# ElenaBiagi/Finito

Hardware: AMD Instinct MI355X
Metric: localized k-mers/s (k=31) (higher is better)
Workload: dtype u32

## Files before the change

### finito_amd/csrc/fin_capi.cpp

```cpp
#include <functional>
#include <hip/hip_runtime_api.h>
#include <sched.h>

#include <algorithm>
#include <atomic>
#include <chrono>
#include <condition_variable>
#include <cstdio>
#include <cstdlib>
#include <cstring>
#include <memory>
#include <mutex>
#include <new>
#include <string>
#include <thread>
#include <vector>

#include "../../include/finito_amd.h"
#include "fin_index.hpp"
#include "fin_kernels.h"

static void set_err(char* err, size_t errlen, const std::string& msg) {
    if (err && errlen) { snprintf(err, errlen, "%s", msg.c_str()); }
}
// ... 28 lines not shown
        if (hipHostMalloc(&p, want, hipHostMallocDefault) != hipSuccess) return nullptr;
        *cap = want;
        return p;
    }
    void put(void* p, size_t cap) {
        if (!p) return;
        {
            std::lock_guard<std::mutex> g(mu);
            if (free_list.size() < 8 && held + cap <= (4ull << 30)) { free_list.push_back({p, cap}); held += cap; return; }
        }
        (void)hipHostFree(p);
    }
    void release_all() {
        std::lock_guard<std::mutex> g(mu);
        for (auto& f : free_list) (void)hipHostFree(f.first);
        free_list.clear(); held = 0;
    }
};
StagePool g_stage;
bool is_page_locked(const void* p) {
    if (!p) return true;
    hipPointerAttribute_t a;
    memset(&a, 0, sizeof a);
    if (hipPointerGetAttributes(&a, p) != hipSuccess) { (void)hipGetLastError(); return false; }
    return a.type == hipMemoryTypeHost;
}
}

extern "C" {

const char* fin_version(void) { return "finito-amd 0.1 (gfx950)"; }

enum : int { O_lds_deque_limit, O_kernel, O_probe_prepass, O_ptab_t, O_jtab_t, O_write_gaps, O_overlap_prefill, O_filt_f, O_seed_anchors, O_kmer_table,
              O_defer_strand, O_fast_path, O_cbf_m, O_lean_tables, O_text_anchors, O_epoch_budget_mult, O_epoch_budget_add, O_max_batch_kmers, O_pipeline_kmers, O_pipeline_depth, O_stage_pageable, O_debug_ovf_cap, O_debug_pp_seg, O_lean_walk, O_fused_ingest, O_pp_park, O_debug_pp_park_cap, O_pp_wide_out, O_hits_combine, O_cover_probe, O_debug_depth_tile, O_ec_tag_bits, O_ec_combine, O_COUNT };
static_assert(O_COUNT <= FIN_N_OPTIONS, "fin_index::opt_val has room for every option");
struct OptDef { const char* name; int64_t def, lo, hi; };
static const OptDef OPTS[O_COUNT] = {
    {"lds_deque_limit", 16, 1, 16},
    {"kernel", 4, 0, 4},
    {"probe_prepass", 1, 0, 1},
    {"ptab_t", -1, -1, 15},
    {"jtab_t", -1, -1, 14},
    {"write_gaps", 1, 0, 1},
    {"overlap_prefill", 1, 0, 1},
    {"filt_f", -1, -1, 16},
    {"seed_anchors", 1, 0, 1},
    {"kmer_table", 1, 0, 1},
    {"defer_strand", 1, 0, 1},
    {"fast_path", 1, 0, 2},
    {"cbf_m", -1, -1, 32},
    {"lean_tables", 2, 0, 3},
    {"text_anchors", 1, 0, 1},
    {"epoch_budget_mult", 64, 0, 64},
    {"epoch_budget_add", 4096, 1, 1 << 20},
    {"max_batch_kmers", 1ll << 30, 1, 1ll << 31},
    {"pipeline_kmers", 1ll << 26, 1, 1ll << 31},
    {"pipeline_depth", 3, 1, 8},
    {"stage_pageable", 1, 0, 1},
    {"debug_ovf_cap", 0, 0, 1ll << 31},
    {"debug_pp_seg", 0, 0, 1024},
    {"lean_walk", 1, 0, 1},
    {"fused_ingest", 1, 0, 1},
    {"pp_park", 1, 0, 1},
    {"debug_pp_park_cap", -1, -1, 1024},
    {"pp_wide_out", 1, 0, 1},
    {"hits_combine", 4, 0, 64},
    {"cover_probe", 0, 0, 1},
    {"debug_depth_tile", 0, 0, 4096},
    {"ec_tag_bits", 63, 1, 63},
    {"ec_combine", 1, 0, 1},
};
static std::atomic<int64_t> g_opt[O_COUNT];
static const bool g_opt_init = [] { for (int i = 0; i < O_COUNT; i++) g_opt[i].store(OPTS[i].def); return true; }();
static inline int64_t optv(const fin_index* x, int id) { return x && x->opt_set[id].load(std::memory_order_acquire) ? x->opt_val[id].load(std::memory_order_relaxed) : g_opt[id].load(std::memory_order_relaxed); }
static int opt_find(const char* name, int64_t value) {
    if (!name) return -1;
    for (int i = 0; i < O_COUNT; i++)
        if (!strcmp(name, OPTS[i].name)) return (value < OPTS[i].lo || value > OPTS[i].hi || (i == O_kernel && value == 1)) ? -1 : i;
    return -1;
}

int fin_set_option(const char* name, int64_t value) {
    (void)g_opt_init;
    const int id = opt_find(name, value);
    if (id < 0) return FIN_EINVAL;
    g_opt[id].store(value);
    if (id == O_stage_pageable && !value) g_stage.release_all();
    return FIN_OK;
}

int fin_index_set_option(fin_index* idx, const char* name, int64_t value) {
    if (!idx) return FIN_EINVAL;
    const int id = opt_find(name, value);
    if (id < 0) return FIN_EINVAL;
    idx->opt_val[id].store(value, std::memory_order_relaxed); idx->opt_set[id].store(true, std::memory_order_release);
    return FIN_OK;
}

// ... 707 lines not shown
    const int rc = batch_load(b, bases ? bases + offsets[0] : nullptr, offsets, n_reads, err, errlen);
    if (rc != FIN_OK) { fin_batch_free(b); return rc; }
    *out = b;
    return FIN_OK;
}

int fin_batch_reload(fin_batch* b, const char* bases, const uint64_t* offsets, uint64_t n_reads, char* err, size_t errlen) {
    if (!b || !offsets || (n_reads && !bases)) { set_err(err, errlen, "null argument"); return FIN_EINVAL; }
    return batch_load(b, bases ? bases + offsets[0] : nullptr, offsets, n_reads, err, errlen);
}

int fin_batch_run(fin_batch* b, int strands, void* hip_stream, char* err, size_t errlen) {
    if (!b || (strands != FIN_FWD && strands != FIN_MERGED)) { set_err(err, errlen, "bad argument"); return FIN_EINVAL; }
    HIPCHK(hipSetDevice(b->device));
    hipStream_t st = (hipStream_t)hip_stream;
    if (b->runs.size() >= 1024) {
        for (auto& e : b->runs.front().e) (void)hipEventDestroy(e);
        b->runs.erase(b->runs.begin());
    }
    fin_batch::RunEvents ev;
    for (auto& e : ev.e) HIPCHK(hipEventCreate(&e));
    b->runs.push_back(ev);
    b->last_strands = strands;
    b->last_stream = st; b->ran = true;
    HIPCHK(hipEventRecord(ev.e[0], st));
    b->dev.budget_mult = (uint32_t)optv(b->idx, O_epoch_budget_mult); b->dev.budget_add = (uint32_t)optv(b->idx, O_epoch_budget_add);
    b->dev.ovf_cap = (uint32_t)std::min<uint64_t>(b->cap_ovf_list / 4, 0xFFFFFFFFull);
    if (const int64_t forced = optv(b->idx, O_debug_ovf_cap)) b->dev.ovf_cap = (uint32_t)std::min<int64_t>(forced, (int64_t)b->dev.ovf_cap);
    b->last_ovf_cap = b->dev.ovf_cap; b->ovf_state = 0; b->rec_ready = false; b->sgm_ready = false; b->rsum_ready = false; b->scr_ready = false; b->cls_ready = false; b->psa_ready = false;
    b->dev.pp_seg = (uint32_t)optv(b->idx, O_debug_pp_seg);
    b->dev.pp_max_len = (uint32_t)std::min<uint64_t>(b->max_read_len, 0xFFFFFFFFull);
    b->dev.pp_park = (uint32_t)optv(b->idx, O_pp_park);
    b->dev.pp_wide_out = (uint32_t)optv(b->idx, O_pp_wide_out);
    b->dev.pp_park_cap = (uint32_t)(int32_t)optv(b->idx, O_debug_pp_park_cap);
    b->dev.lean_walk = (uint32_t)optv(b->idx, O_lean_walk);
    {
        const fin_index::Replica* rep = b->idx->replica_on(b->device);
        b->dev.text_anchors = (optv(b->idx, O_text_anchors) && rep && rep->anchors_built) ? 1u : 0u;
        b->dev.safe = rep ? rep->dev.safe : nullptr;
        b->dev.pos = (optv(b->idx, O_seed_anchors) && b->dev.text_anchors && b->d_seed && rep) ? rep->dev.pos : nullptr;
        b->dev.filt = (optv(b->idx, O_filt_f) != 0 && rep) ? rep->dev.filt : nullptr;
        const bool lean = rep && rep->lean && optv(b->idx, O_seed_anchors) && b->dev.text_anchors && b->d_seed && optv(b->idx, O_kmer_table) && rep->dev.fbf;
        b->dev.fbf = lean ? rep->dev.fbf : nullptr;
        b->dev.kt3 = (optv(b->idx, O_kmer_table) && rep && (b->dev.pos || lean)) ? rep->dev.kt3 : nullptr;
        b->dev.ktx = (b->dev.kt3 && rep) ? rep->dev.ktx : nullptr; b->dev.ktx_log2 = rep ? rep->dev.ktx_log2 : 0;
        b->dev.cbf = (rep && b->dev.kt3) ? rep->dev.cbf : nullptr;
        b->dev.fast_path = (optv(b->idx, O_fast_path) && b->dev.cbf) ? 1u : 0u;
    }
    int rc = 0;
    hipEvent_t out_ready = nullptr;
    const int opt_kernel = (int)optv(b->idx, O_kernel);
    const uint32_t lds_limit = (uint32_t)optv(b->idx, O_lds_deque_limit);
    int kern = opt_kernel;
    if (b->dev.k > FIN_FAST_K)
        kern = (opt_kernel == 4 && b->q_slots && fin_v4_writes_gaps(&b->dev, (const uint32_t*)b->d_seed)) ? 4 : 0;
    const int no_prefill = (kern == 4 && b->q_slots && optv(b->idx, O_write_gaps) && fin_v4_writes_gaps(&b->dev, (const uint32_t*)b->d_seed)) ? 1 : 0;
    {
        const fin_index::Replica* rep = b->idx->replica_on(b->device);
        b->dev.defer_ok = (kern == 4 && no_prefill && strands == FIN_MERGED && optv(b->idx, O_defer_strand) && rep && rep->anchors_built &&
                           rep->n_rc_pairs != ~0ull && (b->dev.pos || b->dev.fbf)) ? 1u : 0u;
        b->dev.rcwin = (b->dev.defer_ok && rep->d_rcwin) ? (const uint8_t*)rep->d_rcwin : nullptr;
    }
    b->last_kernel = (uint32_t)((kern == 4 && !b->q_slots) ? 3 : kern); b->last_no_prefill = (uint32_t)no_prefill;
    if (!(b->dev.defer_ok && b->dev.kt3 && (b->dev.k <= 63 || optv(b->idx, O_fast_path) >= 2))) b->dev.fast_path = 0u;
    b->dev.frec = nullptr; b->dev.text_only = 0u; b->last_frec = false; b->last_text_only = false; b->count_from_text = false;
    if (b->text_mode && kern == 4 && b->q_slots && b->dev.fast_path && no_prefill && strands == FIN_MERGED && b->n_reads) {
// ... 2713 lines not shown
```

### finito_amd/csrc/fin_format.h

```cpp
#pragma once
#include <stdint.h>

#define FIN_BLOCK_NODES 64
#define FIN_LCS_MASK 0x7Fu
#define FIN_USTART_BIT 0x80u
#define FIN_MAX_K 255
#define FIN_FAST_K 128

struct FinCharRec {
    uint32_t plane_lo, plane_hi;
    uint32_t base;
};
struct alignas(128) FinNodeBlock {
    uint8_t node[64];
    FinCharRec rec[4];
    uint64_t th0, th1;
};
static_assert(sizeof(FinNodeBlock) == 128, "one block = one 128-B line");
#ifdef __HIPCC__
__host__ __device__
#endif
static inline uint64_t fin_plane(const FinCharRec& r) { return r.plane_lo | ((uint64_t)r.plane_hi << 32); }

struct FinBlockInfo {
// ... 14 lines not shown
    uint32_t n_nodes;
    uint32_t n_unitigs;
    uint32_t total_len;
    uint32_t k;
    uint32_t samp_shift;
    uint32_t n_samp;
    uint32_t C[5];
    uint32_t lcs_t0;
    uint32_t ptab_t;
    const struct FinPrefixIval* ptab;
    uint32_t jtab_t;
    const struct FinPrefixIval* jtab;
    uint32_t budget_mult, budget_add;
    uint32_t ovf_cap;
    uint32_t text_anchors;
    const struct FinSeedEntry* pos;
    const unsigned long long* safe;
    const struct FinKt3Bucket* kt3;
    uint32_t kt3_buckets;
    const struct FinKtxSlot* ktx;
    uint32_t ktx_log2;
    const struct FinCbfBlock* cbf;
    uint32_t cbf_log2, cbf_m;
    const struct FinCbfBlock* fbf;
    uint32_t fast_path;
    uint32_t defer_ok;
    const uint8_t* rcwin;
    const uint32_t* filt;
    uint32_t filt_f;
    const uint8_t* lcs8;
    struct FinFastRec* frec;
    uint32_t text_only;
    uint32_t pp_wide_out;
    uint32_t lean_walk;
    uint32_t pp_seg;
    uint32_t pp_max_len;
    uint32_t pp_park;
    uint32_t pp_park_cap;
};
struct FinFastRec { uint32_t u, off0, meta, nk; uint64_t Es, Es2; };
struct FinDepthStat { unsigned long long sum; uint32_t max, n_at_least; };
struct FinKt3Bucket { uint32_t w[8]; };
struct FinKtxSlot { uint32_t k0_lo, k0_hi, k1_lo, k1_hi, g, claim, pad0, pad1; };
#define FIN_KT3_SLOTS 4
#define FIN_KT3_TAGMASK 0x3FFFFFFFu
#define FIN_KT3_UNVER 0x40000000u
#define FIN_KT3_EMPTY 0xFFFFFFFFFFFFFFFFull
#define FIN_KT3_LOAD_PCT 55
#ifdef __HIPCC__
__host__ __device__
#endif
static inline uint64_t fin_mix64(uint64_t x) {
    x ^= x >> 29; x *= 0xBF58476D1CE4E5B9ull; x ^= x >> 32; x *= 0x94D049BB133111EBull; x ^= x >> 29;
    return x;
}
#ifdef __HIPCC__
__host__ __device__
#endif
static inline uint64_t fin_kt3_hash(uint64_t k0, uint64_t k1) {
    uint64_t key = k0;
    if (k1) key ^= fin_mix64(k1 + 0x9E3779B97F4A7C15ull);
    return fin_mix64(key);
}
#define FIN_KT3_FOLD 0x9E3779B97F4A7C15ull
#ifdef __HIPCC__
__host__ __device__
// ... 37 lines not shown
```

### finito_amd/csrc/fin_prepass.hip

```cpp
#include <cstdio>
#include <cstring>
#include <type_traits>

#include "fin_device.h"
#include "fin_kernels.h"
#include "fin_pack.h"

#ifndef FIN_V3_PM_ADD
#define FIN_V3_PM_ADD 4
#endif
#define FIN_PP_SEG_MAX 1024

namespace {
constexpr uint32_t NONE = 0xFFFFFFFFu;

struct PpConsts {
    const char* blk_base; const FinPrefixIval* ptab; const uint32_t* filt;
    const FinCbfBlock* fbf; uint32_t fbf_mask;
    uint32_t n, C0, C1, C2, C3, C4, fmask;
    int k, PT, PM, F;
};

__device__ __forceinline__ void pp_window(const uint4& c0, const uint4& c1, int p, uint64_t& w, uint32_t& v) {
    const uint32_t j = (uint32_t)p & 31u;
    const uint64_t b0 = c0.x | ((uint64_t)c0.y << 32), b1 = c1.x | ((uint64_t)c1.y << 32);
    w = b0 >> (2 * j); v = c0.z >> j;
    if (j) { w |= b1 << (64 - 2 * j); v |= c1.z << (32 - j); }
}

__device__ __forceinline__ bool pp_fbf_knows(const PpConsts& K, uint64_t w) {
    const uint64_t f = w & (K.PM >= 32 ? ~0ull : ((1ull << (2 * K.PM)) - 1ull));
    const uint64_t h = fin_cbf_hash(f);
    const uint4 b = *(const uint4*)(K.fbf + ((h >> 35) & K.fbf_mask));
    uint32_t m0 = 0, m1 = 0, m2 = 0, m3 = 0;
#pragma unroll
    for (int i = 0; i < FIN_CBF_BITS; i++) {
        const uint32_t pb = (uint32_t)(h >> (7 * i)) & 127u, bit = 1u << (pb & 31u);
        m0 |= (pb >> 5) == 0u ? bit : 0u; m1 |= (pb >> 5) == 1u ? bit : 0u; m2 |= (pb >> 5) == 2u ? bit : 0u; m3 |= (pb >> 5) == 3u ? bit : 0u;
    }
    return (b.x & m0) == m0 && (b.y & m1) == m1 && (b.z & m2) == m2 && (b.w & m3) == m3;
}

__device__ __forceinline__ bool probe_step(const PpConsts& K, const uint4* chunks, uint32_t r_len, uint32_t& t0, uint32_t& node) {
    const int k = K.k;
    const int span = max(K.PM - 1, K.F);
    const int p0 = (int)t0 - span;
    const int ci0 = p0 >> 5, ci1 = (int)t0 >> 5;
    const uint4 c0 = chunks[ci0];
    uint4 c1 = c0;
    if (ci1 != ci0) c1 = chunks[ci1];
    auto window = [&](int p, uint64_t& w, uint32_t& v) { if ((p >> 5) == ci0) pp_window(c0, c1, p, w, v); else pp_window(c1, c1, p, w, v); };
    if (K.F > 0) {
        uint64_t w; uint32_t v;
        window((int)t0 - K.F, w, v);
        const uint32_t inv = ~v;
        const uint32_t fi = inv ? (uint32_t)(__ffs((int)inv) - 1) : 32u;
        if (fi > (uint32_t)K.F) {
            const uint32_t key0 = (uint32_t)w & K.fmask, key1 = (uint32_t)(w >> 2) & K.fmask;
            const uint32_t w1 = K.filt[key1 >> 5], w0 = K.filt[key0 >> 5];
            uint32_t adv = 0;
            if (!((w1 >> (key1 & 31u)) & 1u)) adv = (uint32_t)(k - K.F + 1);
            else if (!((w0 >> (key0 & 31u)) & 1u)) adv = (uint32_t)(k - K.F);
            if (adv) { t0 += adv; if (t0 >= r_len) t0 = NONE; return false; }
        }
    }
    const int p = (int)t0 - K.PM + 1;
    uint64_t w; uint32_t v;
    window(p, w, v);
    const uint32_t inv = ~v;
    const uint32_t pfi = inv ? (uint32_t)(__ffs((int)inv) - 1) : 32u;
    if (K.fbf) {
        if (pfi >= (uint32_t)K.PM && pp_fbf_knows(K, w)) { node = NONE; return true; }
        t0 = (uint32_t)(p + k);
// ... 207 lines not shown
    const uint64_t wa = a.x | ((uint64_t)a.y << 32), wb = b.x | ((uint64_t)b.y << 32), wc = c.x | ((uint64_t)c.y << 32);
    const uint64_t w0 = o ? (wa >> (2 * o)) | (wb << (64 - 2 * o)) : wa, w1 = o ? (wb >> (2 * o)) | (wc << (64 - 2 * o)) : wb;
    const uint32_t v0 = o ? (a.z >> o) | (b.z << (32 - o)) : a.z, v1 = o ? (b.z >> o) | (c.z << (32 - o)) : b.z;
    const uint32_t n1 = k - 32u;
    const uint32_t need1 = n1 ? (1u << n1) - 1u : 0u;
    if (v0 != 0xFFFFFFFFu || (v1 & need1) != need1) return false;
    return kt3_find(ix, w0, n1 ? w1 & ((1ull << (2 * n1)) - 1ull) : 0ull, g_ans, verified);
}

template <typename CH>
__device__ __forceinline__ bool look_ktabN_at(const FinDevIndex& ix, const CH& ch, uint32_t t, uint32_t r_len, uint32_t& g_ans, bool& verified) {
    const uint32_t k = ix.k, p = t - (k - 1u), j0 = p >> 5, o = p & 31u, jl = (r_len - 1u) >> 5, nw = (k + 31u) >> 5;
    uint4 a = ch[j0];
    uint64_t key = 0;
    for (uint32_t w = 0; w < nw; w++) {
        const uint4 b = ch[j0 + w + 1u <= jl ? j0 + w + 1u : jl];
        const uint64_t wa = a.x | ((uint64_t)a.y << 32), wb = b.x | ((uint64_t)b.y << 32);
        uint64_t word = o ? (wa >> (2u * o)) | (wb << (64u - 2u * o)) : wa;
        const uint32_t valid = o ? (a.z >> o) | (b.z << (32u - o)) : a.z;
        const uint32_t nb = k - 32u * w < 32u ? k - 32u * w : 32u;
        const uint32_t need = nb == 32u ? 0xFFFFFFFFu : (1u << nb) - 1u;
        if ((valid & need) != need) return false;
        if (nb < 32u) word &= (1ull << (2u * nb)) - 1ull;
        key = w == 0u ? word : fin_kt3_fold(key, word, w);
        a = b;
    }
    return kt3_find_h(ix, fin_mix64(key), g_ans, verified);
}

#define FIN_FAST_MAXE 4
#ifdef FIN_PP_STATS
__device__ unsigned long long g_fin_ppdbg[16];
#define PPDBG(i) atomicAdd(&g_fin_ppdbg[i], 1ull)
#else
#define PPDBG(i) ((void)0)
#endif
typedef uint32_t fin_u4 __attribute__((ext_vector_type(4)));
struct FastRun { uint32_t ok, u, off0, nE; uint64_t Es, Es2; };

struct StrandChunks {
    const uint64_t* row; uint32_t stride, len, ok; bool rev;
    __device__ __forceinline__ uint4 operator[](uint32_t j) const {
        const uint32_t q = len - 32u * j, o = ok - 32u * j;
        const uint32_t cnt = (int)o <= 0 ? 0u : (o < q ? o : q) < 32u ? (o < q ? o : q) : 32u;
        uint64_t w;
        if (!rev) w = row[j * stride];
        else {
            uint64_t x;
            if (q >= 32u) {
                const uint32_t p = q - 32u, a = p >> 5, sh = p & 31u;
                x = row[a * stride] >> (2u * sh);
                if (sh) x |= row[(a + 1u) * stride] << (64u - 2u * sh);
            } else x = row[0] << (64u - 2u * q);
            w = fin_pack::revcomp32(x);
        }
        if (cnt < 32u) w &= (1ull << (2u * cnt)) - 1ull;
        return make_uint4((uint32_t)w, (uint32_t)(w >> 32), cnt < 32u ? (1u << cnt) - 1u : 0xFFFFFFFFu, 0u);
    }
};
__device__ __forceinline__ bool row_holds(const uint4*) { return false; }
__device__ __forceinline__ bool row_holds(const StrandChunks&) { return true; }
__device__ __forceinline__ bool row_mirrored(const uint4*) { return false; }
__device__ __forceinline__ bool row_mirrored(const StrandChunks& c) { return c.rev; }
__device__ __forceinline__ const uint64_t* ask_row(const uint4*, const uint64_t* lds, uint32_t& stride) { stride = FIN_TPB; return lds; }
__device__ __forceinline__ const uint64_t* ask_row(const StrandChunks& c, const uint64_t*, uint32_t& stride) { stride = c.stride; return c.row; }

__device__ __forceinline__ uint64_t pp_revcomp(uint64_t f, uint32_t m, uint64_t mask) {
    uint64_t r = __brevll(f);
    r = ((r >> 1) & 0x5555555555555555ull) | ((r & 0x5555555555555555ull) << 1);
    return (r >> (64u - 2u * m)) ^ mask;
}
struct CbfAsk { uint4 blk; uint32_t mw[4]; };
__device__ __forceinline__ void cbf_ask(const FinDevIndex& ix, const uint64_t* lds, uint32_t ls, uint32_t a, uint32_t m, uint64_t mask, CbfAsk& q) {
    const uint32_t j = a >> 5, o = a & 31u;
    uint64_t w = lds[j * ls] >> (2 * o);
    if (o + m > 32u) w |= lds[(j + 1) * ls] << (64u - 2u * o);
    const uint64_t f = w & mask, v = pp_revcomp(f, m, mask);
    const uint64_t h = fin_cbf_hash(f < v ? f : v);
    q.blk = *(const uint4*)(ix.cbf + ((h >> 35) & ((1ull << ix.cbf_log2) - 1ull)));
    q.mw[0] = q.mw[1] = q.mw[2] = q.mw[3] = 0u;
#pragma unroll
    for (int i = 0; i < FIN_CBF_BITS; i++) {
        const uint32_t p = (uint32_t)(h >> (7 * i)) & 127u, bit = 1u << (p & 31u);
        q.mw[0] |= (p >> 5) == 0u ? bit : 0u; q.mw[1] |= (p >> 5) == 1u ? bit : 0u; q.mw[2] |= (p >> 5) == 2u ? bit : 0u; q.mw[3] |= (p >> 5) == 3u ? bit : 0u;
    }
}
__device__ __forceinline__ bool cbf_known(const CbfAsk& q) {
    return (q.blk.x & q.mw[0]) == q.mw[0] && (q.blk.y & q.mw[1]) == q.mw[1] && (q.blk.z & q.mw[2]) == q.mw[2] && (q.blk.w & q.mw[3]) == q.mw[3];
}
template <typename CH>
__device__ __forceinline__ bool fast_try(const PpConsts& K, const FinDevIndex& ix, const CH& ch, uint32_t t_anchor, uint32_t r_len, uint32_t g_ans, uint64_t* lds, FastRun& res) {
    const uint32_t k = (uint32_t)K.k, m = ix.cbf_m;
    const bool put = !row_holds(ch), mir = row_mirrored(ch);
    uint32_t ls;
    const uint64_t* const arow = ask_row(ch, lds, ls);
    const uint32_t nch = (r_len + 31u) >> 5;
    if (nch > FIN_FAST_CHUNKS || g_ans < t_anchor) { PPDBG(1); return false; }
    const uint32_t gs = g_ans - t_anchor;
    uint32_t u, ustart, uend;
    {
        uint32_t idx = ix.samp[gs >> ix.samp_shift];
        uint4 e4; __builtin_memcpy(&e4, ix.ends + idx, 16);
        while (e4.w <= gs) { idx += 3u; __builtin_memcpy(&e4, ix.ends + idx, 16); }
        if (gs < e4.y) { u = idx; ustart = e4.x; uend = e4.y; }
        else if (gs < e4.z) { u = idx + 1u; ustart = e4.y; uend = e4.z; }
        else { u = idx + 2u; ustart = e4.z; uend = e4.w; }
    }
    if (gs < ustart || gs + r_len > uend) { PPDBG(2); return false; }
    const uint64_t* const text = (const uint64_t*)ix.concat;
    const uint32_t tw = gs >> 5, sh = (gs & 31u) * 2u;
    uint64_t Es = 0, Es2 = 0; uint32_t nE = 0; bool bad = false;
    auto E_at = [&](uint32_t e) -> uint32_t { return (uint32_t)((e < 4u ? Es : Es2) >> (16u * (e & 3u))) & 0xFFFFu; };
    uint64_t w0 = text[tw];
    for (uint32_t jb = 0; jb < nch; jb += 4u) {
        uint4 c[4]; uint64_t tx[4];
#pragma unroll
        for (uint32_t i = 0; i < 4u; i++) {
            const uint32_t j = jb + i < nch ? jb + i : nch - 1u;
            c[i] = ch[j]; tx[i] = text[tw + j + 1u];
        }
#pragma unroll
        for (uint32_t i = 0; i < 4u; i++) {
            const uint32_t j = jb + i;
            if (j < nch) {
                const uint64_t w1 = tx[i];
                const uint64_t tb = sh ? (w0 >> sh) | (w1 << (64u - sh)) : w0;
                w0 = w1;
                const uint64_t rb = c[i].x | ((uint64_t)c[i].y << 32);
                if (put) lds[j * FIN_TPB] = rb;
                const uint32_t nb = r_len - 32u * j < 32u ? r_len - 32u * j : 32u;
                const uint32_t vm = nb == 32u ? 0xFFFFFFFFu : (1u << nb) - 1u;
                bad = bad || (c[i].z & vm) != vm;
                const uint64_t x = rb ^ tb;
                uint64_t y = (x | (x >> 1)) & 0x5555555555555555ull;
                if (nb < 32u) y &= (1ull << (2u * nb)) - 1ull;
                while (y && nE < FIN_FAST_MAXE) {
                    const uint32_t p = (uint32_t)(__ffsll((long long)y) - 1) >> 1;
                    y &= y - 1ull;
                    if (nE < 4u) Es |= (uint64_t)(32u * j + p) << (16u * nE); else Es2 |= (uint64_t)(32u * j + p) << (16u * (nE - 4u));
                    nE++;
                }
                bad = bad || y != 0ull;
            }
        }
    }
    if (bad) { PPDBG(3); return false; }
    if (ix.rcwin) {
        for (uint32_t w = (gs + k - 1u) >> 6; w <= (gs + r_len - 1u) >> 6; w++) if ((ix.rcwin[w >> 3] >> (w & 7u)) & 1u) { PPDBG(5); return false; }
    }
    if (ix.safe && t_anchor != k - 1u && (nE == 0u || E_at(0) >= k) && !((ix.safe[(gs + k - 1u) >> 6] >> ((gs + k - 1u) & 63u)) & 1ull)) { PPDBG(7); return false; }
    const uint64_t mask = m >= 32u ? ~0ull : ((1ull << (2u * m)) - 1ull);
    uint32_t covered = k - 2u;
    bool known = false, unsafe = false;
    for (uint32_t e = 0; e < nE; e++) {
        const uint32_t E = E_at(e);
        uint32_t lo = E > k - 1u ? E : k - 1u; if (lo < covered + 1u) lo = covered + 1u;
        const uint32_t hi = E + k - 1u < r_len - 1u ? E + k - 1u : r_len - 1u;
        CbfAsk q0, q1, q2; bool h0 = false, h1 = false, h2 = false;
        if (lo <= hi) { const uint32_t a = lo - (m - 1u) < E ? lo - (m - 1u) : E; cbf_ask(ix, arow, ls, mir ? r_len - a - m : a, m, mask, q0); h0 = true; covered = a + k - 1u; lo = covered + 1u; }
        if (lo <= hi) { const uint32_t a = lo - (m - 1u) < E ? lo - (m - 1u) : E; cbf_ask(ix, arow, ls, mir ? r_len - a - m : a, m, mask, q1); h1 = true; covered = a + k - 1u; lo = covered + 1u; }
        if (lo <= hi) { const uint32_t a = lo - (m - 1u) < E ? lo - (m - 1u) : E; cbf_ask(ix, arow, ls, mir ? r_len - a - m : a, m, mask, q2); h2 = true; covered = a + k - 1u; lo = covered + 1u; }
        const uint32_t t = E + k;
        const bool last = e + 1u == nE || E_at(e + 1u) > t;
        unsigned long long sw = ~0ull;
        if (ix.safe && last && t < r_len) sw = ix.safe[(gs + t) >> 6];
        known = known || (h0 && cbf_known(q0)) || (h1 && cbf_known(q1)) || (h2 && cbf_known(q2)) || lo <= hi;
        unsafe = unsafe || !((sw >> ((gs + t) & 63u)) & 1ull);
    }
    if (known) { PPDBG(6); return false; }
    if (unsafe) { PPDBG(7); return false; }
    PPDBG(0);
    res.ok = 1u; res.u = u; res.off0 = gs - ustart; res.nE = nE; res.Es = Es; res.Es2 = Es2;
    return true;
}
template <typename CH>
__device__ __forceinline__ bool fast_all_absent(const PpConsts& K, const FinDevIndex& ix, const CH& ch, uint32_t r_len, uint64_t* lds) {
    const uint32_t k = (uint32_t)K.k, m = ix.cbf_m;
    const uint32_t nch = (r_len + 31u) >> 5;
    if (nch > FIN_FAST_CHUNKS) return false;
    if constexpr (std::is_same<CH, StrandChunks>::value) {
        if (ch.ok < r_len) return false;
    } else {
        bool bad = false;
        for (uint32_t j = 0; j < nch; j++) {
            const uint4 c = ch[j];
            const uint32_t nb = r_len - 32u * j < 32u ? r_len - 32u * j : 32u;
            const uint32_t vm = nb == 32u ? 0xFFFFFFFFu : (1u << nb) - 1u;
            bad = bad || (c.z & vm) != vm;
            lds[j * FIN_TPB] = c.x | ((uint64_t)c.y << 32);
        }
        if (bad) return false;
    }
    uint32_t ls;
    const uint64_t* const arow = ask_row(ch, lds, ls);
    const uint64_t mask = m >= 32u ? ~0ull : ((1ull << (2u * m)) - 1ull);
    bool known = false;
    for (uint32_t t = k - 1u; t < r_len; ) {
        CbfAsk q[4]; bool h[4];
#pragma unroll
        for (int i = 0; i < 4; i++) { h[i] = t < r_len; const uint32_t a = (h[i] ? t : k - 1u) - (m - 1u); cbf_ask(ix, arow, ls, a, m, mask, q[i]); if (h[i]) t = a + k; }
#pragma unroll
        for (int i = 0; i < 4; i++) known = known || (h[i] && cbf_known(q[i]));
        if (known) break;
    }
    if (known) { PPDBG(10); return false; }
    PPDBG(11);
// ... 129 lines not shown
                const bool v_hit = probe_step(K, cv, r_len, v_t0, sd.y);
                if (v_hit && can_defer && f_t0 != NONE) f_t0 = FIN_PASS_DEFERRED;
            }
            verdict = make_uint2(f_t0, v_t0);
        }
        *(uint2*)(pass + 2 * (size_t)r) = verdict;
        if (seed) *(uint2*)(seed + 2 * (size_t)r) = sd;
        if (!is_final(verdict.x) || !is_final(verdict.y)) to_tail(r);
    };
    for (uint32_t rb = r_lo; rb < r_hi; rb += FIN_TPB) {
        const uint32_t r = rb + threadIdx.x;
        FinReadDesc d = {0, 0, 0};
        if (r < r_hi) d = desc[r];
        const uint32_t r_len = d.len, r_nch = (r_len + 31u) >> 5;
        typename std::conditional<FUSED, StrandChunks, const uint4*>::type cf, cv;
        bool acgt = true;
        if constexpr (FUSED) {
            uint64_t* const row = ck + threadIdx.x;
            const uint8_t* const rd = bases + (r < r_hi ? offs[r] : 0ull);
            uint32_t fi = r_len, li = NONE;
            for (uint32_t j = 0; j < r_nch; j++) {
                uint64_t c; uint32_t v;
                fin_pack::make_chunk(rd, r_len, j, false, c, v);
                row[j * FIN_TPB] = c;
                const uint32_t cnt = r_len - 32u * j;
                const uint32_t inv = ~v & (cnt < 32u ? (1u << cnt) - 1u : 0xFFFFFFFFu);
                if (inv) { if (fi == r_len) fi = 32u * j + (uint32_t)(__ffs((int)inv) - 1); li = 32u * j + 31u - (uint32_t)__clz((int)inv); }
            }
            cf = StrandChunks{row, FIN_TPB, r_len, fi, false}; cv = StrandChunks{row, FIN_TPB, r_len, li == NONE ? r_len : r_len - 1u - li, true};
            acgt = li == NONE;
        } else { cf = packed + d.off; cv = cf + r_nch; }
        uint2 verdict = make_uint2(NONE, NONE), sd = make_uint2(NONE, NONE);
        FastRun fr = {0u, 0u, 0u, 0u, 0ull, 0ull}; bool fr_rev = false, to_a = false, parked = false;
        auto to_list_a = [&]() {
            const uint32_t ia = atomicAdd(&lds_na, 1u);
            lds_list[ia] = (uint16_t)(r - r_lo);
            if constexpr (FUSED) {
                if (ia < cap) {
                    parked = acgt;
                    park_len[ia] = parked ? (uint16_t)r_len : (uint16_t)0u;
                    if (parked) {
                        park_out[ia] = d.out_off;
                        for (uint32_t j = 0; j < r_nch; j++) park[j * cap + ia] = cf.row[j * FIN_TPB];
                    }
                }
            }
        };
        auto count_parked = [&]() {
            if constexpr (FUSED) { const uint64_t mp = __ballot(parked); if (lane == 0 && mp) atomicAdd(&lds_np, (uint32_t)__popcll(mp)); }
        };
        auto spill = [&]() {
            if constexpr (FUSED) {
                if (r < r_hi && !fr.ok && !parked) {
                    if (acgt) for (uint32_t j = 0; j < r_nch; j++) { packed_out[d.off + j] = cf[j]; packed_out[d.off + r_nch + j] = cv[j]; }
                    else for (uint32_t j = 0; j < 2u * r_nch; j++) {
                        uint64_t c; uint32_t v;
                        fin_pack::make_chunk(bases + offs[r], r_len, j < r_nch ? j : j - r_nch, j >= r_nch, c, v);
                        packed_out[d.off + j] = make_uint4((uint32_t)c, (uint32_t)(c >> 32), v, 0u);
                    }
                }
            }
        };
        if (KT2) {
            if (r < r_hi) {
                bool hit = false, settled = false;
                if (r_len >= (uint32_t)K.k && defer && r_len < 65536u) {
                    uint32_t g_f = NONE, g_v = NONE; bool ver_f = false, ver_v = false;
                    const bool f_hit = flook(cf, k1, r_len, g_f, ver_f);
                    const bool v_hit = !f_hit && flook(cv, k1, r_len, g_v, ver_v);
                    hit = f_hit || v_hit;
                    if (((f_hit && ver_f) || (v_hit && ver_v)) && fast_try(K, ix, v_hit ? cv : cf, k1, r_len, v_hit ? g_v : g_f, ck + threadIdx.x, fr)) fr_rev = v_hit;
                    if (fr.ok) *(uint2*)(pass + 2 * (size_t)r) = make_uint2(FIN_PASS_DONE, FIN_PASS_DONE);
                    else if (!hit) to_list_a();
                    else if (K.fbf) {
                        const uint32_t other = (uint32_t)K.k < r_len ? FIN_PASS_DEFERRED : NONE;
                        *(uint2*)(pass + 2 * (size_t)r) = f_hit ? make_uint2(k1, FIN_PASS_DEFERRED) : make_uint2(other, k1);
                        if (seed) *(uint2*)(seed + 2 * (size_t)r) = make_uint2((f_hit && ver_f && pp_claim_holds<!FUSED>(ix, cf, g_f)) ? g_f : NONE, (v_hit && ver_v && pp_claim_holds<!FUSED>(ix, cv, g_v)) ? g_v : NONE);
                        settled = true;
                    }
                }
                if (!fr.ok && !settled && (hit || !(r_len >= (uint32_t)K.k && defer && r_len < 65536u))) to_l(r);
            }
            spill();
            count_parked();
            write_out(fr, fr_rev, r, d.out_off, r_len);
            continue;
        }
        if (r < r_hi && r_len >= (uint32_t)K.k) {
            const bool can_defer = defer && r_len < 65536u;
            const uint32_t after = (uint32_t)K.k < r_len ? (uint32_t)K.k : NONE;
            uint32_t f_t0 = k1, v_t0 = k1;
            if (look_kt) {
                uint32_t g_f = NONE, g_v = NONE; bool ver_f = false, ver_v = false, v_hit = false;
                const bool f_hit = look_ktab(K, ix, cf[0], g_f, ver_f);
                sd.x = (f_hit && ver_f) ? g_f : NONE;
                if (!f_hit) f_t0 = after;
                if (f_hit && can_defer) v_t0 = FIN_PASS_DEFERRED;
                else {
                    v_hit = look_ktab(K, ix, cv[0], g_v, ver_v);
                    sd.y = (v_hit && ver_v) ? g_v : NONE;
                    if (!v_hit) v_t0 = after;
                    if (v_hit && can_defer && f_t0 != NONE) f_t0 = FIN_PASS_DEFERRED;
                }
                if (FAST && can_defer) {
                    const bool af = f_hit && ver_f, av = !f_hit && v_hit && ver_v;
                    if ((af || av) && fast_try(K, ix, av ? cv : cf, k1, r_len, av ? g_v : g_f, ck + threadIdx.x, fr)) fr_rev = av;
                    if ((f_hit && !ver_f) || (!f_hit && v_hit && !ver_v)) PPDBG(8);
                    to_a = !f_hit && !v_hit;
                    if (to_a) PPDBG(9);
                }
            } else if constexpr (!FUSED) {
                const bool f_hit = probe_step(K, cf, r_len, f_t0, sd.x);
                if (f_hit && can_defer) v_t0 = FIN_PASS_DEFERRED;
                else {
                    const bool v_hit = probe_step(K, cv, r_len, v_t0, sd.y);
                    if (v_hit && can_defer && f_t0 != NONE) f_t0 = FIN_PASS_DEFERRED;
                }
            }
            if (look_kt && !fr.ok) {
                if (sd.x != NONE && !pp_claim_holds<!FUSED>(ix, cf, sd.x)) sd.x = NONE;
                if (sd.y != NONE && !pp_claim_holds<!FUSED>(ix, cv, sd.y)) sd.y = NONE;
            }
            verdict = fr.ok ? make_uint2(FIN_PASS_DONE, FIN_PASS_DONE) : make_uint2(f_t0, v_t0);
        }
        if (r < r_hi) {
            *(uint2*)(pass + 2 * (size_t)r) = verdict;
            if (seed) *(uint2*)(seed + 2 * (size_t)r) = sd;
            if (to_a) to_list_a();
            else if (!is_final(verdict.x) || !is_final(verdict.y)) lds_list[FIN_PP_SEG_MAX - 1u - atomicAdd(&lds_n, 1u)] = (uint16_t)(r - r_lo);
        }
        spill();
        count_parked();
        if (FAST) write_out(fr, fr_rev, r, d.out_off, r_len);
    }
    __syncthreads();
    if constexpr (FUSED) {
        if (threadIdx.x == 0 && n_fast) {
            if (lds_np) atomicAdd(n_fast + 1, lds_np);
            if (lds_na > cap) atomicAdd(n_fast + 2, lds_na - cap);
        }
    }
    if (FAST) {
        const uint32_t n_a = lds_na;
        auto park_chunks = [&](uint32_t i, uint32_t r_len, bool rev) { return StrandChunks{park + i, cap, r_len, r_len, rev}; };
        auto spill_parked = [&](uint32_t i, uint32_t r) {
            if constexpr (FUSED) {
                const FinReadDesc d = desc[r];
                const uint32_t r_nch = (d.len + 31u) >> 5;
                const StrandChunks f = park_chunks(i, d.len, false), v = park_chunks(i, d.len, true);
                for (uint32_t j = 0; j < r_nch; j++) { packed_out[d.off + j] = f[j]; packed_out[d.off + r_nch + j] = v[j]; }
            }
// ... 166 lines not shown
    uint32_t seg = (n_reads + grid_hint - 1) / (grid_hint ? grid_hint : 1u);
    seg = (seg + FIN_TPB - 1) / FIN_TPB * FIN_TPB;
    if (seg > FIN_PP_SEG_MAX) seg = FIN_PP_SEG_MAX;
    if (n_reads >= 512u * FIN_PP_SEG_MAX) seg = FIN_PP_SEG_MAX;
    if (ix->pp_seg >= FIN_TPB && ix->pp_seg <= FIN_PP_SEG_MAX && ix->pp_seg % FIN_TPB == 0) seg = ix->pp_seg;
    const int fast = (out && defer) ? pp_fast_kernel(ix) : 0;
    const dim3 grid((n_reads + seg - 1) / seg);
    if (bases && (!fast || !offs || ix->k > 63)) return (int)hipErrorInvalidValue;
    if (bases) {
        uint32_t rch, cap;
        const void* const kern = fast == 2 ? (const void*)fin_fast2_prepass_fused_kernel : (const void*)fin_fast_prepass_fused_kernel;
        const size_t dyn = pp_fused_lds(ix, kern, seg, rch, cap);
        if (rch > FIN_FAST_CHUNKS) return (int)hipErrorInvalidValue;
        if (fast == 2)
            hipLaunchKernelGGL(fin_fast2_prepass_fused_kernel, grid, dim3(FIN_TPB), dyn, stream, *ix, (uint4*)packed, desc, n_reads, seg, pass, seed, defer, (int2*)out, n_fast, bases, offs, rch, cap);
        else
            hipLaunchKernelGGL(fin_fast_prepass_fused_kernel, grid, dim3(FIN_TPB), dyn, stream, *ix, (uint4*)packed, desc, n_reads, seg, pass, seed, defer, (int2*)out, n_fast, bases, offs, rch, cap);
    } else if (fast == 2)
        hipLaunchKernelGGL(fin_fast2_prepass_kernel, grid, dim3(FIN_TPB), 0, stream, *ix, (const uint4*)packed, desc, n_reads, seg, pass, seed, defer, (int2*)out, n_fast);
    else if (fast == 1)
        hipLaunchKernelGGL(fin_fast_prepass_kernel, grid, dim3(FIN_TPB), 0, stream, *ix, (const uint4*)packed, desc, n_reads, seg, pass, seed, defer, (int2*)out, n_fast);
    else
        hipLaunchKernelGGL(fin_pair_prepass_kernel, grid, dim3(FIN_TPB), 0, stream, *ix, (const uint4*)packed, desc, n_reads, seg, pass, seed, defer);
    return (int)hipGetLastError();
}

extern "C" void fin_debug_dump_pp(void) {
#ifdef FIN_PP_STATS
    unsigned long long h[16];
    (void)hipDeviceSynchronize();
    (void)hipMemcpyFromSymbol(h, HIP_SYMBOL(g_fin_ppdbg), sizeof h);
    fprintf(stderr, "[fin_ppdbg] fast ok %llu | too long / no answer %llu  unitig ends inside %llu  non-ACGT %llu  > %d errors %llu  rc window %llu  filter knows %llu  unsafe place %llu | unverified %llu  both first looks fail %llu | all-absent: a string known %llu  proven %llu\n",
            h[0], h[1], h[2], h[3], FIN_FAST_MAXE, h[4], h[5], h[6], h[7], h[8], h[9], h[10], h[11]);
    memset(h, 0, sizeof h);
    (void)hipMemcpyToSymbol(HIP_SYMBOL(g_fin_ppdbg), h, sizeof h);
#endif
}
```

Measured before the change: 216.6 billion.

## Add wave-cooperative CBF ask scheduling behind pp_wave_asks option, simplify bloom check

Adds an optional mode, off by default, in which fast_try only records its planned counting-Bloom-filter asks per lane. A wave-wide prefix sum then spreads those asks evenly across all 64 lanes, so lanes with few errors no longer sit idle while others loop. The block membership test is also rewritten to check bits directly from two 64-bit halves instead of building four masks. The default path only gets the simpler bit test and some restructured control flow around the new settle step.

```diff
diff --git a/finito_amd/csrc/fin_capi.cpp b/finito_amd/csrc/fin_capi.cpp
--- a/finito_amd/csrc/fin_capi.cpp
+++ b/finito_amd/csrc/fin_capi.cpp
@@ -84,7 +84,7 @@
 const char* fin_version(void) { return "finito-amd 0.1 (gfx950)"; }
 
 enum : int { O_lds_deque_limit, O_kernel, O_probe_prepass, O_ptab_t, O_jtab_t, O_write_gaps, O_overlap_prefill, O_filt_f, O_seed_anchors, O_kmer_table,
-              O_defer_strand, O_fast_path, O_cbf_m, O_lean_tables, O_text_anchors, O_epoch_budget_mult, O_epoch_budget_add, O_max_batch_kmers, O_pipeline_kmers, O_pipeline_depth, O_stage_pageable, O_debug_ovf_cap, O_debug_pp_seg, O_lean_walk, O_fused_ingest, O_pp_park, O_debug_pp_park_cap, O_pp_wide_out, O_hits_combine, O_cover_probe, O_debug_depth_tile, O_ec_tag_bits, O_ec_combine, O_COUNT };
+              O_defer_strand, O_fast_path, O_cbf_m, O_lean_tables, O_text_anchors, O_epoch_budget_mult, O_epoch_budget_add, O_max_batch_kmers, O_pipeline_kmers, O_pipeline_depth, O_stage_pageable, O_debug_ovf_cap, O_debug_pp_seg, O_lean_walk, O_fused_ingest, O_pp_park, O_debug_pp_park_cap, O_pp_wide_out, O_pp_wave_asks, O_hits_combine, O_cover_probe, O_debug_depth_tile, O_ec_tag_bits, O_ec_combine, O_COUNT };
 static_assert(O_COUNT <= FIN_N_OPTIONS, "fin_index::opt_val has room for every option");
 struct OptDef { const char* name; int64_t def, lo, hi; };
 static const OptDef OPTS[O_COUNT] = {
@@ -116,6 +116,7 @@
     {"pp_park", 1, 0, 1},
     {"debug_pp_park_cap", -1, -1, 1024},
     {"pp_wide_out", 1, 0, 1},
+    {"pp_wave_asks", 0, 0, 1},
     {"hits_combine", 4, 0, 64},
     {"cover_probe", 0, 0, 1},
     {"debug_depth_tile", 0, 0, 4096},
@@ -889,6 +890,7 @@
     b->dev.pp_max_len = (uint32_t)std::min<uint64_t>(b->max_read_len, 0xFFFFFFFFull);
     b->dev.pp_park = (uint32_t)optv(b->idx, O_pp_park);
     b->dev.pp_wide_out = (uint32_t)optv(b->idx, O_pp_wide_out);
+    b->dev.pp_wave_asks = (uint32_t)optv(b->idx, O_pp_wave_asks);
     b->dev.pp_park_cap = (uint32_t)(int32_t)optv(b->idx, O_debug_pp_park_cap);
     b->dev.lean_walk = (uint32_t)optv(b->idx, O_lean_walk);
     {
diff --git a/finito_amd/csrc/fin_format.h b/finito_amd/csrc/fin_format.h
--- a/finito_amd/csrc/fin_format.h
+++ b/finito_amd/csrc/fin_format.h
@@ -70,6 +70,7 @@
     struct FinFastRec* frec;
     uint32_t text_only;
     uint32_t pp_wide_out;
+    uint32_t pp_wave_asks;
     uint32_t lean_walk;
     uint32_t pp_seg;
     uint32_t pp_max_len;
diff --git a/finito_amd/csrc/fin_prepass.hip b/finito_amd/csrc/fin_prepass.hip
--- a/finito_amd/csrc/fin_prepass.hip
+++ b/finito_amd/csrc/fin_prepass.hip
@@ -28,17 +28,21 @@
     if (j) { w |= b1 << (64 - 2 * j); v |= c1.z << (32 - j); }
 }
 
+__device__ __forceinline__ bool pp_block_has(const uint4& b, uint64_t h) {
+    const uint64_t lo = b.x | ((uint64_t)b.y << 32), hi = b.z | ((uint64_t)b.w << 32);
+    uint32_t all = 1u;
+#pragma unroll
+    for (int i = 0; i < FIN_CBF_BITS; i++) {
+        const uint32_t p = (uint32_t)(h >> (7 * i)) & 127u;
+        all &= (uint32_t)(((p & 64u) ? hi : lo) >> (p & 63u));
+    }
+    return (all & 1u) != 0u;
+}
 __device__ __forceinline__ bool pp_fbf_knows(const PpConsts& K, uint64_t w) {
     const uint64_t f = w & (K.PM >= 32 ? ~0ull : ((1ull << (2 * K.PM)) - 1ull));
     const uint64_t h = fin_cbf_hash(f);
     const uint4 b = *(const uint4*)(K.fbf + ((h >> 35) & K.fbf_mask));
-    uint32_t m0 = 0, m1 = 0, m2 = 0, m3 = 0;
-#pragma unroll
-    for (int i = 0; i < FIN_CBF_BITS; i++) {
-        const uint32_t pb = (uint32_t)(h >> (7 * i)) & 127u, bit = 1u << (pb & 31u);
-        m0 |= (pb >> 5) == 0u ? bit : 0u; m1 |= (pb >> 5) == 1u ? bit : 0u; m2 |= (pb >> 5) == 2u ? bit : 0u; m3 |= (pb >> 5) == 3u ? bit : 0u;
-    }
-    return (b.x & m0) == m0 && (b.y & m1) == m1 && (b.z & m2) == m2 && (b.w & m3) == m3;
+    return pp_block_has(b, h);
 }
 
 __device__ __forceinline__ bool probe_step(const PpConsts& K, const uint4* chunks, uint32_t r_len, uint32_t& t0, uint32_t& node) {
@@ -312,6 +316,7 @@
 #ifdef FIN_PP_STATS
 __device__ unsigned long long g_fin_ppdbg[16];
 #define PPDBG(i) atomicAdd(&g_fin_ppdbg[i], 1ull)
+#define PPDBG_ADD(i, v) atomicAdd(&g_fin_ppdbg[i], (unsigned long long)(v))
 #else
 #define PPDBG(i) ((void)0)
 #endif
@@ -350,7 +355,7 @@
     r = ((r >> 1) & 0x5555555555555555ull) | ((r & 0x5555555555555555ull) << 1);
     return (r >> (64u - 2u * m)) ^ mask;
 }
-struct CbfAsk { uint4 blk; uint32_t mw[4]; };
+struct CbfAsk { uint4 blk; uint64_t h; };
 __device__ __forceinline__ void cbf_ask(const FinDevIndex& ix, const uint64_t* lds, uint32_t ls, uint32_t a, uint32_t m, uint64_t mask, CbfAsk& q) {
     const uint32_t j = a >> 5, o = a & 31u;
     uint64_t w = lds[j * ls] >> (2 * o);
@@ -358,18 +363,13 @@
     const uint64_t f = w & mask, v = pp_revcomp(f, m, mask);
     const uint64_t h = fin_cbf_hash(f < v ? f : v);
     q.blk = *(const uint4*)(ix.cbf + ((h >> 35) & ((1ull << ix.cbf_log2) - 1ull)));
-    q.mw[0] = q.mw[1] = q.mw[2] = q.mw[3] = 0u;
-#pragma unroll
-    for (int i = 0; i < FIN_CBF_BITS; i++) {
-        const uint32_t p = (uint32_t)(h >> (7 * i)) & 127u, bit = 1u << (p & 31u);
-        q.mw[0] |= (p >> 5) == 0u ? bit : 0u; q.mw[1] |= (p >> 5) == 1u ? bit : 0u; q.mw[2] |= (p >> 5) == 2u ? bit : 0u; q.mw[3] |= (p >> 5) == 3u ? bit : 0u;
-    }
-}
-__device__ __forceinline__ bool cbf_known(const CbfAsk& q) {
-    return (q.blk.x & q.mw[0]) == q.mw[0] && (q.blk.y & q.mw[1]) == q.mw[1] && (q.blk.z & q.mw[2]) == q.mw[2] && (q.blk.w & q.mw[3]) == q.mw[3];
-}
-template <typename CH>
-__device__ __forceinline__ bool fast_try(const PpConsts& K, const FinDevIndex& ix, const CH& ch, uint32_t t_anchor, uint32_t r_len, uint32_t g_ans, uint64_t* lds, FastRun& res) {
+    q.h = h;
+}
+__device__ __forceinline__ bool cbf_known(const CbfAsk& q) { return pp_block_has(q.blk, q.h); }
+struct AskPlan { uint64_t A0s; uint32_t meta; };
+static_assert(FIN_FAST_MAXE <= 4, "AskPlan: four starts of 16 bits, four counts of 2 bits");
+template <bool DEFER = false, typename CH>
+__device__ __forceinline__ bool fast_try(const PpConsts& K, const FinDevIndex& ix, const CH& ch, uint32_t t_anchor, uint32_t r_len, uint32_t g_ans, uint64_t* lds, FastRun& res, AskPlan* pl = nullptr) {
     const uint32_t k = (uint32_t)K.k, m = ix.cbf_m;
     const bool put = !row_holds(ch), mir = row_mirrored(ch);
     uint32_t ls;
@@ -432,26 +432,102 @@
     const uint64_t mask = m >= 32u ? ~0ull : ((1ull << (2u * m)) - 1ull);
     uint32_t covered = k - 2u;
     bool known = false, unsafe = false;
+    uint64_t A0s = 0ull; uint32_t cnts = 0u;
+#ifdef FIN_PP_STATS
+    if constexpr (!DEFER) {
+        const uint64_t act = __ballot(1);
+        uint32_t trips = 0;
+        for (uint32_t e = 0; e < FIN_FAST_MAXE; e++) if (__ballot(nE > e)) trips = e + 1u;
+        if ((threadIdx.x & 63u) == (uint32_t)(__ffsll((long long)act) - 1)) { PPDBG(12); PPDBG_ADD(13, __popcll(act)); PPDBG_ADD(14, trips); }
+    }
+#endif
     for (uint32_t e = 0; e < nE; e++) {
         const uint32_t E = E_at(e);
         uint32_t lo = E > k - 1u ? E : k - 1u; if (lo < covered + 1u) lo = covered + 1u;
         const uint32_t hi = E + k - 1u < r_len - 1u ? E + k - 1u : r_len - 1u;
         CbfAsk q0, q1, q2; bool h0 = false, h1 = false, h2 = false;
-        if (lo <= hi) { const uint32_t a = lo - (m - 1u) < E ? lo - (m - 1u) : E; cbf_ask(ix, arow, ls, mir ? r_len - a - m : a, m, mask, q0); h0 = true; covered = a + k - 1u; lo = covered + 1u; }
-        if (lo <= hi) { const uint32_t a = lo - (m - 1u) < E ? lo - (m - 1u) : E; cbf_ask(ix, arow, ls, mir ? r_len - a - m : a, m, mask, q1); h1 = true; covered = a + k - 1u; lo = covered + 1u; }
-        if (lo <= hi) { const uint32_t a = lo - (m - 1u) < E ? lo - (m - 1u) : E; cbf_ask(ix, arow, ls, mir ? r_len - a - m : a, m, mask, q2); h2 = true; covered = a + k - 1u; lo = covered + 1u; }
+        uint32_t a0 = 0u;
+        if (lo <= hi) { const uint32_t a = lo - (m - 1u) < E ? lo - (m - 1u) : E; if constexpr (!DEFER) cbf_ask(ix, arow, ls, mir ? r_len - a - m : a, m, mask, q0); a0 = a; h0 = true; covered = a + k - 1u; lo = covered + 1u; }
+        if (lo <= hi) { const uint32_t a = lo - (m - 1u) < E ? lo - (m - 1u) : E; if constexpr (!DEFER) cbf_ask(ix, arow, ls, mir ? r_len - a - m : a, m, mask, q1); h1 = true; covered = a + k - 1u; lo = covered + 1u; }
+        if (lo <= hi) { const uint32_t a = lo - (m - 1u) < E ? lo - (m - 1u) : E; if constexpr (!DEFER) cbf_ask(ix, arow, ls, mir ? r_len - a - m : a, m, mask, q2); h2 = true; covered = a + k - 1u; lo = covered + 1u; }
+#ifdef FIN_PP_STATS
+        PPDBG_ADD(15, (uint32_t)h0 + (uint32_t)h1 + (uint32_t)h2);
+#endif
         const uint32_t t = E + k;
         const bool last = e + 1u == nE || E_at(e + 1u) > t;
         unsigned long long sw = ~0ull;
         if (ix.safe && last && t < r_len) sw = ix.safe[(gs + t) >> 6];
+        if constexpr (DEFER) {
+            A0s |= (uint64_t)a0 << (16u * e); cnts |= ((uint32_t)h0 + (uint32_t)h1 + (uint32_t)h2) << (2u * e);
+            known = known || lo <= hi;
+        } else
         known = known || (h0 && cbf_known(q0)) || (h1 && cbf_known(q1)) || (h2 && cbf_known(q2)) || lo <= hi;
         unsafe = unsafe || !((sw >> ((gs + t) & 63u)) & 1ull);
+    }
+    if constexpr (DEFER) {
+        pl->A0s = A0s; pl->meta = cnts | ((uint32_t)mir << 8) | ((uint32_t)known << 9) | ((uint32_t)unsafe << 10) | (r_len << 16);
+        res.ok = 1u; res.u = u; res.off0 = gs - ustart; res.nE = nE; res.Es = Es; res.Es2 = Es2;
+        return true;
     }
     if (known) { PPDBG(6); return false; }
     if (unsafe) { PPDBG(7); return false; }
     PPDBG(0);
     res.ok = 1u; res.u = u; res.off0 = gs - ustart; res.nE = nE; res.Es = Es; res.Es2 = Es2;
     return true;
+}
+__device__ __forceinline__ uint32_t pp_lane_of(uint32_t v, uint32_t l) { return (uint32_t)__builtin_amdgcn_ds_bpermute((int)(l << 2), (int)v); }
+__device__ __forceinline__ bool wave_asks(const FinDevIndex& ix, const uint64_t* rows, uint32_t ls, uint32_t k, uint32_t lane, const AskPlan& pl, uint64_t Es) {
+    const uint32_t m = ix.cbf_m, step = k - m + 1u;
+    const uint64_t mask = m >= 32u ? ~0ull : ((1ull << (2u * m)) - 1ull);
+    const uint32_t cn = pl.meta & 0xFFu;
+    uint32_t incl = (cn & 3u) + ((cn >> 2) & 3u) + ((cn >> 4) & 3u) + (cn >> 6);
+#pragma unroll
+    for (uint32_t d = 1; d < 64u; d <<= 1) { const uint32_t v = __shfl_up(incl, d, 64); if (lane >= d) incl += v; }
+    const uint32_t total = (uint32_t)__builtin_amdgcn_readlane((int)incl, 63);
+    bool known = false;
+    __builtin_amdgcn_fence(__ATOMIC_RELEASE, "wavefront");
+    __builtin_amdgcn_wave_barrier();
+    for (uint32_t base = 0; base < total; base += 128u) {
+        CbfAsk q[2]; uint32_t own[2] = {NONE, NONE};
+#pragma unroll
+        for (uint32_t u = 0; u < 2u; u++) {
+            if (base + 64u * u < total) {
+                const uint32_t n0 = base + 64u * u + lane, n = n0 < total ? n0 : total - 1u;
+                uint32_t o = 0;
+#pragma unroll
+                for (uint32_t s = 32u; s; s >>= 1) if (pp_lane_of(incl, o + s - 1u) <= n) o += s;
+                const uint32_t o_incl = pp_lane_of(incl, o), o_meta = pp_lane_of(pl.meta, o);
+                const uint64_t o_A0 = pp_lane_of((uint32_t)pl.A0s, o) | ((uint64_t)pp_lane_of((uint32_t)(pl.A0s >> 32), o) << 32);
+                const uint64_t o_Es = pp_lane_of((uint32_t)Es, o) | ((uint64_t)pp_lane_of((uint32_t)(Es >> 32), o) << 32);
+                const uint32_t c0 = o_meta & 3u, c1 = (o_meta >> 2) & 3u, c2 = (o_meta >> 4) & 3u, c3 = (o_meta >> 6) & 3u;
+                uint32_t j = n - (o_incl - (c0 + c1 + c2 + c3)), e = 0;
+                if (j >= c0) { j -= c0; e = 1u; if (j >= c1) { j -= c1; e = 2u; if (j >= c2) { j -= c2; e = 3u; } } }
+                const uint32_t E = (uint32_t)(o_Es >> (16u * e)) & 0xFFFFu, a0 = (uint32_t)(o_A0 >> (16u * e)) & 0xFFFFu;
+                uint32_t a = a0 + j * step < E ? a0 + j * step : E;
+                if (o_meta & 0x100u) a = (o_meta >> 16) - a - m;
+                cbf_ask(ix, rows + o, ls, a, m, mask, q[u]);
+                if (n0 < total) own[u] = o;
+            }
+        }
+#pragma unroll
+        for (uint32_t u = 0; u < 2u; u++) {
+            if (base + 64u * u < total) {
+                uint64_t km = __ballot(own[u] != NONE && cbf_known(q[u]));
+                while (km) {
+                    const int src = __ffsll((long long)km) - 1;
+                    km &= km - 1ull;
+                    if (lane == (uint32_t)__builtin_amdgcn_readlane((int)own[u], src)) known = true;
+                }
+            }
+        }
+    }
+    return known;
+}
+__device__ __forceinline__ void fast_settle(FastRun& fr, bool& fr_rev, const AskPlan& pl, bool known) {
+    if (!fr.ok) return;
+    const bool kn = known || (pl.meta & 0x200u), us = (pl.meta & 0x400u) != 0u;
+    if (kn) PPDBG(6); else if (us) PPDBG(7); else PPDBG(0);
+    if (kn || us) { fr = FastRun{0u, 0u, 0u, 0u, 0ull, 0ull}; fr_rev = false; }
 }
 template <typename CH>
 __device__ __forceinline__ bool fast_all_absent(const PpConsts& K, const FinDevIndex& ix, const CH& ch, uint32_t r_len, uint64_t* lds) {
@@ -647,6 +723,19 @@
         } else { cf = packed + d.off; cv = cf + r_nch; }
         uint2 verdict = make_uint2(NONE, NONE), sd = make_uint2(NONE, NONE);
         FastRun fr = {0u, 0u, 0u, 0u, 0ull, 0ull}; bool fr_rev = false, to_a = false, parked = false;
+        AskPlan pl = {0ull, 0u};
+        auto attempt = [&](const auto& ch, uint32_t g) -> bool {
+            if constexpr (FUSED && !KT2) { if (ix.pp_wave_asks) return fast_try<true>(K, ix, ch, k1, r_len, g, ck + threadIdx.x, fr, &pl); }
+            return fast_try(K, ix, ch, k1, r_len, g, ck + threadIdx.x, fr);
+        };
+        auto settle = [&]() {
+            if constexpr (FUSED && !KT2) {
+                if (ix.pp_wave_asks) {
+                    const bool kn = wave_asks(ix, ck + (threadIdx.x - lane), FIN_TPB, (uint32_t)K.k, lane, pl, fr.Es);
+                    fast_settle(fr, fr_rev, pl, kn);
+                }
+            }
+        };
         auto to_list_a = [&]() {
             const uint32_t ia = atomicAdd(&lds_na, 1u);
             lds_list[ia] = (uint16_t)(r - r_lo);
@@ -677,14 +766,18 @@
             }
         };
         if (KT2) {
+            const bool looks = r < r_hi && r_len >= (uint32_t)K.k && defer && r_len < 65536u;
+            uint32_t g_f = NONE, g_v = NONE; bool ver_f = false, ver_v = false, f_hit = false, v_hit = false;
+            if (looks) {
+                f_hit = flook(cf, k1, r_len, g_f, ver_f);
+                v_hit = !f_hit && flook(cv, k1, r_len, g_v, ver_v);
+                if (((f_hit && ver_f) || (v_hit && ver_v)) && attempt(v_hit ? cv : cf, v_hit ? g_v : g_f)) fr_rev = v_hit;
+            }
+            settle();
             if (r < r_hi) {
-                bool hit = false, settled = false;
-                if (r_len >= (uint32_t)K.k && defer && r_len < 65536u) {
-                    uint32_t g_f = NONE, g_v = NONE; bool ver_f = false, ver_v = false;
-                    const bool f_hit = flook(cf, k1, r_len, g_f, ver_f);
-                    const bool v_hit = !f_hit && flook(cv, k1, r_len, g_v, ver_v);
-                    hit = f_hit || v_hit;
-                    if (((f_hit && ver_f) || (v_hit && ver_v)) && fast_try(K, ix, v_hit ? cv : cf, k1, r_len, v_hit ? g_v : g_f, ck + threadIdx.x, fr)) fr_rev = v_hit;
+                const bool hit = f_hit || v_hit;
+                bool settled = false;
+                if (looks) {
                     if (fr.ok) *(uint2*)(pass + 2 * (size_t)r) = make_uint2(FIN_PASS_DONE, FIN_PASS_DONE);
                     else if (!hit) to_list_a();
                     else if (K.fbf) {
@@ -694,17 +787,18 @@
                         settled = true;
                     }
                 }
-                if (!fr.ok && !settled && (hit || !(r_len >= (uint32_t)K.k && defer && r_len < 65536u))) to_l(r);
+                if (!fr.ok && !settled && (hit || !looks)) to_l(r);
             }
             spill();
             count_parked();
             write_out(fr, fr_rev, r, d.out_off, r_len);
             continue;
         }
-        if (r < r_hi && r_len >= (uint32_t)K.k) {
+        const bool has_kmer = r < r_hi && r_len >= (uint32_t)K.k;
+        uint32_t f_t0 = k1, v_t0 = k1;
+        if (has_kmer) {
             const bool can_defer = defer && r_len < 65536u;
             const uint32_t after = (uint32_t)K.k < r_len ? (uint32_t)K.k : NONE;
-            uint32_t f_t0 = k1, v_t0 = k1;
             if (look_kt) {
                 uint32_t g_f = NONE, g_v = NONE; bool ver_f = false, ver_v = false, v_hit = false;
                 const bool f_hit = look_ktab(K, ix, cf[0], g_f, ver_f);
@@ -719,7 +813,7 @@
                 }
                 if (FAST && can_defer) {
                     const bool af = f_hit && ver_f, av = !f_hit && v_hit && ver_v;
-                    if ((af || av) && fast_try(K, ix, av ? cv : cf, k1, r_len, av ? g_v : g_f, ck + threadIdx.x, fr)) fr_rev = av;
+                    if ((af || av) && attempt(av ? cv : cf, av ? g_v : g_f)) fr_rev = av;
                     if ((f_hit && !ver_f) || (!f_hit && v_hit && !ver_v)) PPDBG(8);
                     to_a = !f_hit && !v_hit;
                     if (to_a) PPDBG(9);
@@ -732,6 +826,9 @@
                     if (v_hit && can_defer && f_t0 != NONE) f_t0 = FIN_PASS_DEFERRED;
                 }
             }
+        }
+        if (FAST) settle();
+        if (has_kmer) {
             if (look_kt && !fr.ok) {
                 if (sd.x != NONE && !pp_claim_holds<!FUSED>(ix, cf, sd.x)) sd.x = NONE;
                 if (sd.y != NONE && !pp_claim_holds<!FUSED>(ix, cv, sd.y)) sd.y = NONE;
@@ -964,6 +1061,7 @@
     (void)hipMemcpyFromSymbol(h, HIP_SYMBOL(g_fin_ppdbg), sizeof h);
     fprintf(stderr, "[fin_ppdbg] fast ok %llu | too long / no answer %llu  unitig ends inside %llu  non-ACGT %llu  > %d errors %llu  rc window %llu  filter knows %llu  unsafe place %llu | unverified %llu  both first looks fail %llu | all-absent: a string known %llu  proven %llu\n",
             h[0], h[1], h[2], h[3], FIN_FAST_MAXE, h[4], h[5], h[6], h[7], h[8], h[9], h[10], h[11]);
+    fprintf(stderr, "[fin_ppdbg] the per-lane ask loop: wave passes %llu  lanes in them %llu  trips %llu  strings asked %llu\n", h[12], h[13], h[14], h[15]);
     memset(h, 0, sizeof h);
     (void)hipMemcpyToSymbol(HIP_SYMBOL(g_fin_ppdbg), h, sizeof h);
 #endif
```

Result: no change. 216.4 billion, median of 2 (-0.1%).
